# vincentjzy/OpenCorr

Hardware: AMD Instinct MI355X
Metric: converged POIs/sec (FFTCC+ICGN2D1, 33x33 subset) (higher is better)
Workload: dtype f32

## Files before the change

opencorr_amd/csrc/capi.hip:

```cpp
#include "capi_internal.h"

namespace ochip_capi {

thread_local std::string g_last_error;

int fail(int code, const char* fmt, ...) {
    char buf[512];
    va_list ap;
    va_start(ap, fmt);
    vsnprintf(buf, sizeof(buf), fmt, ap);
    va_end(ap);
    g_last_error = buf;
    return code;
}

static std::once_flag g_rocfft_once;
void rocfft_init_once() {
    std::call_once(g_rocfft_once, [] { rocfft_setup(); });
}

int create_engine(int kind, int rx, int ry, int rz, float conv, float stop, int device, oc_hip_engine** out) {
    if (!out) return fail(OC_HIP_ERR_INVALID, "null output handle");
    *out = nullptr;
    if (rx < 1 || ry < 1 || ((kind == OC_HIP_FFTCC3D || kind == OC_HIP_ICGN3D1) && rz < 1))
        return fail(OC_HIP_ERR_INVALID, "subset radius must be >= 1 (got %d, %d, %d)", rx, ry, rz);
    int ndev = 0;
    hipError_t err = hipGetDeviceCount(&ndev);
    if (err != hipSuccess || ndev <= 0)
        return fail(OC_HIP_ERR_HIP, "no usable HIP device: %s", err == hipSuccess ? "device count is 0" : hipGetErrorString(err));
    if (device < 0 || device >= ndev) return fail(OC_HIP_ERR_INVALID, "device %d out of range [0,%d)", device, ndev);
    DeviceScope device_scope;
    OC_HIP_TRY(hipSetDevice(device));
    std::unique_ptr<oc_hip_engine> e(new oc_hip_engine);
    e->kind = kind;
    e->device = device;
    e->rx = rx;
    e->ry = ry;
    e->rz = rz;
    e->conv = conv;
    e->stop = stop;
    OC_HIP_TRY(hipStreamCreateWithFlags(&e->own_stream, hipStreamNonBlocking));
    e->stream = e->own_stream;
    *out = e.release();
    return OC_HIP_OK;
}

}

namespace {

size_t fftcc_chunk_limit() {
#if OC_BUILD_AB
    const char* s = getenv("OC_HIP_FFTCC_CHUNK");
    if (s && *s) {
        long v = atol(s);
        if (v > 0) return (size_t)v;
    }
#endif
    return 32768;
}

int ensure_fft(oc_hip_engine* e, size_t chunk) {
    const int n0 = 2 * e->rx, n1 = 2 * e->ry, n2 = e->is3d() ? 2 * e->rz : 0;
    FftPlans& f = e->fft;
    if (f.fwd && f.n0 == n0 && f.n1 == n1 && f.n2 == n2 && f.chunk == chunk) return OC_HIP_OK;
    rocfft_init_once();
    f.destroy();
    const size_t lengths2[2] = {(size_t)n1, (size_t)n0};
    const size_t lengths3[3] = {(size_t)n2, (size_t)n1, (size_t)n0};
    const size_t* lengths = n2 ? lengths3 : lengths2;
    const size_t dims = n2 ? 3 : 2;
    OC_FFT_TRY(rocfft_plan_create(&f.fwd, rocfft_placement_notinplace, rocfft_transform_type_real_forward,
                                  rocfft_precision_single, dims, lengths, 2 * chunk, nullptr));
    OC_FFT_TRY(rocfft_plan_create(&f.inv, rocfft_placement_notinplace, rocfft_transform_type_real_inverse,
                                  rocfft_precision_single, dims, lengths, chunk, nullptr));
    OC_FFT_TRY(rocfft_execution_info_create(&f.info_fwd));
    OC_FFT_TRY(rocfft_execution_info_create(&f.info_inv));
    size_t wf = 0, wi = 0;
    OC_FFT_TRY(rocfft_plan_get_work_buffer_size(f.fwd, &wf));
    OC_FFT_TRY(rocfft_plan_get_work_buffer_size(f.inv, &wi));
    if (wf) {
        OC_TRY(f.work_fwd.reserve(wf));
        OC_FFT_TRY(rocfft_execution_info_set_work_buffer(f.info_fwd, f.work_fwd.p, wf));
    }
    if (wi) {
        OC_TRY(f.work_inv.reserve(wi));
        OC_FFT_TRY(rocfft_execution_info_set_work_buffer(f.info_inv, f.work_inv.p, wi));
    }
    f.n0 = n0;
    f.n1 = n1;
    f.n2 = n2;
    f.chunk = chunk;
    return OC_HIP_OK;
}

int run_fftcc2d(oc_hip_engine* e, float* d_pois, int stride_f, size_t count) {
    if (!e->img || e->img->ndim != 2) return fail(OC_HIP_ERR_INVALID, "FFTCC2D: set_images2d has not been called");
    const ImagePair& im = *e->img;
    const bool fused32 = e->fftcc2d_fused != 2 && ochip::fftcc2d_fused_supported(e->rx, e->ry);
    const bool rect = ochip::fftcc2d_rect_supported(e->rx, e->ry);
    if (e->fftcc2d_fused && (fused32 || rect || ochip::fftcc2d_fusedn_supported(e->rx, e->ry))) {
        ochip::Fftcc2dParams P = {im.ref_ptr(), im.tar_ptr(), im.dy, im.dx, e->rx, e->ry};
        ProfScope prof(e);
        const size_t kMaxBatch = 1u << 30;
        for (size_t first = 0; first < count; first += kMaxBatch) {
            const size_t n = (count - first) < kMaxBatch ? (count - first) : kMaxBatch;
            float* q = d_pois + first * (size_t)stride_f;
            hipError_t err = fused32 ? ochip::launch_fftcc2d_fused(P, q, stride_f, n, e->icgn2d_xcd != 0, e->stream)
                             : rect  ? ochip::launch_fftcc2d_rect(P, q, stride_f, n, e->icgn2d_xcd != 0, e->stream)
                                     : ochip::launch_fftcc2d_fusedn(P, q, stride_f, n, e->icgn2d_xcd != 0, e->stream);
            if (err != hipSuccess) return fail(OC_HIP_ERR_HIP, "fused FFTCC2D launch failed: %s", hipGetErrorString(err));
        }
        return OC_HIP_OK;
    }
    const size_t chunk = count < fftcc_chunk_limit() ? count : fftcc_chunk_limit();
    if (chunk == 0) return OC_HIP_OK;
    OC_TRY(ensure_fft(e, chunk));
    const size_t M = (size_t)4 * e->rx * e->ry;
    const size_t F = (size_t)(2 * e->rx) * (size_t)(e->ry + 1);
    OC_TRY(e->win.reserve(2 * chunk * M * sizeof(float)));
    OC_TRY(e->freq.reserve(2 * chunk * F * sizeof(float2)));
    OC_TRY(e->norms.reserve(2 * chunk * sizeof(float)));
    OC_TRY(e->flags.reserve(chunk * sizeof(int)));
    OC_FFT_TRY(rocfft_execution_info_set_stream(e->fft.info_fwd, e->stream));
    OC_FFT_TRY(rocfft_execution_info_set_stream(e->fft.info_inv, e->stream));
    ochip::Fftcc2dParams P = {im.ref_ptr(), im.tar_ptr(), im.dy, im.dx, e->rx, e->ry};
    float* ref_win = e->win.as<float>();
    float* tar_win = ref_win + chunk * M;
    float2* ref_freq = e->freq.as<float2>();
    float2* tar_freq = ref_freq + chunk * F;
    ProfScope prof(e);
    for (size_t first = 0; first < count; first += chunk) {
        const size_t n = (count - first) < chunk ? (count - first) : chunk;
        float* pois = d_pois + first * (size_t)stride_f;
        if (n < chunk) {
            OC_HIP_TRY(hipMemsetAsync(ref_win + n * M, 0, (chunk - n) * M * sizeof(float), e->stream));
            OC_HIP_TRY(hipMemsetAsync(tar_win + n * M, 0, (chunk - n) * M * sizeof(float), e->stream));
        }
        OC_HIP_TRY(ochip::launch_fftcc2d_gather(P, pois, stride_f, n, ref_win, tar_win, e->norms.as<float>(),
                                                e->flags.as<int>(), e->stream));
        void* in_fwd[1] = {ref_win};
        void* out_fwd[1] = {ref_freq};
        OC_FFT_TRY(rocfft_execute(e->fft.fwd, in_fwd, out_fwd, e->fft.info_fwd));
        OC_HIP_TRY(ochip::launch_fftcc_conjmul(ref_freq, tar_freq, ref_freq, n * F, e->stream));
        void* in_inv[1] = {ref_freq};
        void* out_inv[1] = {ref_win};
        OC_FFT_TRY(rocfft_execute(e->fft.inv, in_inv, out_inv, e->fft.info_inv));
        OC_HIP_TRY(ochip::launch_fftcc2d_argmax(P, ref_win, e->norms.as<float>(), e->flags.as<int>(), pois, stride_f,
                                                n, e->stream));
    }
    return OC_HIP_OK;
}

int tile_order(oc_hip_engine* e, const float* pois, int stride_f, size_t n, const unsigned** perm, unsigned* xy_copy = nullptr,
               unsigned* xy_word = nullptr, unsigned xy_epoch = 0) {
    *perm = nullptr;
    if (e->icgn2d_tile_px <= 0 || n < 16384) {
        if (xy_copy) OC_HIP_TRY(ochip::launch_poi2d_xy_check(pois, stride_f, n, xy_copy, xy_word, xy_epoch, e->stream));
        return OC_HIP_OK;
    }
    const ImagePair& im = *e->img;
    OC_TRY(e->perm.reserve(n * sizeof(unsigned)));
    OC_TRY(e->tiles.reserve(ochip::poi2d_tile_count(im.dy, im.dx, e->icgn2d_tile_px) * sizeof(unsigned)));
    OC_TRY(e->perm_slots.reserve(n * sizeof(unsigned)));
    OC_HIP_TRY(ochip::launch_poi2d_tile_order(pois, stride_f, n, im.dy, im.dx, e->icgn2d_tile_px, e->tiles.as<unsigned>(),
                                              e->perm_slots.as<unsigned>(), e->perm.as<unsigned>(), e->stream, xy_copy, xy_word, xy_epoch));
    *perm = e->perm.as<unsigned>();
    return OC_HIP_OK;
}

int check_image2d_limits(const char* who, const ImagePair& im, unsigned long long max_pixels) {
    if ((unsigned long long)im.dy * (unsigned long long)im.dx > max_pixels || im.dx >= (1 << 22) || im.dy >= (1 << 22))
        return fail(OC_HIP_ERR_UNSUPPORTED, "%s: image %d x %d exceeds the engine's limit of %llu pixels (width, height < 2^22)", who,
                    im.dx, im.dy, max_pixels);
    return OC_HIP_OK;
}

int run_icgn2d(oc_hip_engine* e, float* d_pois, int stride_f, size_t count, const float* d_offsets) {
    if (!e->img || e->img->ndim != 2) return fail(OC_HIP_ERR_INVALID, "ICGN2D: set_images2d has not been called");
    if (!e->ref_ready || !e->tar_ready)
        return fail(OC_HIP_ERR_INVALID, "ICGN2D: prepare() has not been called since the last set_images");
    const ImagePair& im = *e->img;
    OC_TRY(check_image2d_limits("ICGN2D", im, 1ull << 28));
    const int dof = (e->kind == OC_HIP_ICGN2D1 || e->kind == OC_HIP_ICLM2D1) ? 6 : 12;
    const bool lm = e->is_iclm();
    const bool onepass = e->arith_onepass && !lm;
    if (onepass && d_offsets)
        return fail(OC_HIP_ERR_UNSUPPORTED, "ICGN2D%d: centre offsets are not supported under arith_onepass = 1 (the one-pass kernel keeps "
                                            "integer local coordinates in a per-workgroup table); set arith_onepass = 0 for this call", dof == 6 ? 1 : 2);
    if (onepass && e->self_adaptive)
        return fail(OC_HIP_ERR_UNSUPPORTED, "ICGN2D%d: self-adaptive subset radii are not supported under arith_onepass = 1 (the one-pass "
// ... 736 lines not shown
        }
        if (e->switch_ev && hipEventRecord(e->switch_ev, e->own_stream) == hipSuccess) have_event = true;
        else (void)hipStreamSynchronize(e->own_stream);
    } else {
        have_event = e->tail_marked && e->switch_ev;
    }
    if (have_event && next != e->own_stream) {
        const hipError_t err = hipStreamWaitEvent(next, e->switch_ev, 0);
        if (err != hipSuccess) {
            (void)hipGetLastError();
            return fail(OC_HIP_ERR_HIP, "set_stream: cannot enqueue on the new stream: %s", hipGetErrorString(err));
        }
    } else if (have_event) {
        if (hipStreamWaitEvent(e->own_stream, e->switch_ev, 0) != hipSuccess) {
            (void)hipGetLastError();
            (void)hipEventSynchronize(e->switch_ev);
            (void)hipGetLastError();
        }
    }
    (void)must_succeed;
    e->stream = next;
    e->tail_marked = have_event;
    return OC_HIP_OK;
}

int oc_hip_set_stream(oc_hip_engine* e, void* hip_stream) {
    OC_ACTIVATE(e);
    std::lock_guard<std::mutex> lock(e->mu);
    return switch_stream(e, reinterpret_cast<hipStream_t>(hip_stream), false);
}

int oc_hip_reset_stream(oc_hip_engine* e) {
    OC_ACTIVATE(e);
    std::lock_guard<std::mutex> lock(e->mu);
    return switch_stream(e, e->own_stream, true);
}

int oc_hip_set_tuning(oc_hip_engine* e, const char* key, int value) {
    OC_TRY(check_engine(e));
    if (!key) return fail(OC_HIP_ERR_INVALID, "null tuning key");
    std::lock_guard<std::mutex> lock(e->mu);
    const std::string k(key);
    if (k == "icgn2d_variant") {
        if (value < -1 || value >= ochip::icgn2d_variant_count())
            return fail(OC_HIP_ERR_INVALID, "icgn2d_variant %d out of range [-1 (automatic), %d)", value, ochip::icgn2d_variant_count());
        if (value >= 0 && !ochip::icgn2d_variant_built(value))
            return fail(OC_HIP_ERR_UNSUPPORTED, "icgn2d_variant %d is an A/B partner that only the A/B build of the library contains "
                                               "(python -m opencorr_amd.build --ab)", value);
        e->icgn2d_variant = value;
    } else if (k == "icgn2d_xcd" || k == "xcd") {
        e->icgn2d_xcd = value != 0;
    } else if (k == "arith_fma") {
        if (value != 0 && !(e->is_icgn2d() || e->kind == OC_HIP_ICGN3D1))
            return fail(OC_HIP_ERR_UNSUPPORTED, "arith_fma: only the ICGN2D1 / ICGN2D2 / ICLM2D1 / ICLM2D2 / ICGN3D1 engines have a fused-arithmetic build");
        e->arith_fma = value != 0;
    } else if (k == "arith_onepass") {
        if (value != 0 && e->kind == OC_HIP_ICGN3D1)
            return fail(OC_HIP_ERR_UNSUPPORTED, "arith_onepass: the key of the ICGN2D1 / ICGN2D2 engines; the one-pass build of ICGN3D1 has a "
                                                "key of its own, arith_onepass3d");
        if (value != 0 && !(e->kind == OC_HIP_ICGN2D1 || e->kind == OC_HIP_ICGN2D2))
            return fail(OC_HIP_ERR_UNSUPPORTED, "arith_onepass: only the ICGN2D1 / ICGN2D2 engines have a one-pass build");
        e->arith_onepass = value != 0;
    } else if (k == "arith_onepass3d") {
        if (value != 0 && e->kind != OC_HIP_ICGN3D1)
            return fail(OC_HIP_ERR_UNSUPPORTED, "arith_onepass3d: only the ICGN3D1 engine has this one-pass build (ICGN2D1 / ICGN2D2: "
                                                "arith_onepass)");
        e->arith_onepass3d = value != 0;
    } else if (k == "icgn2d_split_chunks") {
#if !OC_BUILD_AB
        if (value != 0)
            return fail(OC_HIP_ERR_UNSUPPORTED, "icgn2d_split_chunks belongs to icgn2d_variant 8, an A/B partner that only the A/B build of the "
                                                "library contains (python -m opencorr_amd.build --ab)");
#endif
        if (value < 0 || value > 256) return fail(OC_HIP_ERR_INVALID, "icgn2d_split_chunks must be 0 (back to back) ... 256");
        e->icgn2d_split_chunks = value;
    } else if (k == "icgn2d_setup_cache") {
        e->icgn2d_setup_cache = value != 0;
    } else if (k == "icgn2d_int_first") {
        e->icgn2d_int_first = value != 0;
    } else if (k == "icgn2d_tile_px") {
        if (value < 0 || (value > 0 && value < 16)) return fail(OC_HIP_ERR_INVALID, "icgn2d_tile_px must be 0 (off) or >= 16");
        e->icgn2d_tile_px = value;
    } else if (k == "fftcc2d_fused") {
        e->fftcc2d_fused = value == 2 ? 2 : (value != 0);
    } else if (k == "fftcc3d_fused") {
#if !OC_BUILD_AB
        if (value == 2)
            return fail(OC_HIP_ERR_UNSUPPORTED, "fftcc3d_fused = 2 (the 32^3 kernel of rounds 1 - 5) is an A/B partner that only the A/B build of the "
                                                "library contains (python -m opencorr_amd.build --ab)");
#endif
        e->fftcc3d_fused = value == 2 ? 2 : (value != 0);
    } else if (k == "fftcc3d_tile_vox") {
        if (value < 0 || (value > 0 && value < 8)) return fail(OC_HIP_ERR_INVALID, "fftcc3d_tile_vox must be 0 (off) or >= 8");
        e->fftcc3d_tile_vox = value;
    } else if (k == "icgn3d_tile_vox") {
        if (value < 0 || (value > 0 && value < 8)) return fail(OC_HIP_ERR_INVALID, "icgn3d_tile_vox must be 0 (off) or >= 8");
        e->icgn3d_tile_vox = value;
    } else if (k == "icgn3d_mapping") {
#if !OC_BUILD_AB
        if (value != 0)
            return fail(OC_HIP_ERR_UNSUPPORTED, "icgn3d_mapping = 1 (the row mapping, measured 12 - 25 %% slower) is an A/B partner that only "
                                               "the A/B build of the library contains (python -m opencorr_amd.build --ab)");
#endif
        e->icgn3d_mapping = value != 0;
    } else if (k == "fftcc3d_planes_blocks") {
        if (value < 0 || value > 4096) return fail(OC_HIP_ERR_INVALID, "fftcc3d_planes_blocks must be 0 (default) ... 4096");
        e->fftcc3d_planes_blocks = value;
    } else if (k == "single_combine") {
        e->single_combine = value != 0;
    } else if (k == "host_chunk") {
        if (value < 0 || (value > 0 && value < 16384)) return fail(OC_HIP_ERR_INVALID, "host_chunk must be 0 (off) or >= 16384 POIs");
        e->host_chunk = value;
    } else if (k == "group_allgather") {
        e->group_allgather = value != 0;
    } else if (k == "group_force_rccl") {
        e->group_force_rccl = value != 0;
    } else {
        return fail(OC_HIP_ERR_INVALID, "unknown tuning key '%s'", key);
    }
    for (oc_hip_engine* r : e->replicas) OC_TRY(oc_hip_set_tuning(r, key, value));
    return OC_HIP_OK;
}

int oc_hip_prepare_ref(oc_hip_engine* e) {
    OC_ACTIVATE(e);
    if (!e->is_icgn()) return OC_HIP_OK;
    if (!e->img) return fail(OC_HIP_ERR_INVALID, "prepare: set_images has not been called");
    std::lock_guard<std::mutex> lock(e->mu);
    TailGuard tail(e);
    OC_TRY(order_after_default_stream(e));
    const ImagePair& im = *e->img;
    const size_t bytes = im.count() * sizeof(float);
    if (e->kind == OC_HIP_NR2D1) {
        e->ref_ready = true;
        for (oc_hip_engine* r : e->replicas) OC_TRY(oc_hip_prepare_ref(r));
        return OC_HIP_OK;
    }
    if (im.ndim == 2) {
        OC_TRY(e->gx.reserve(bytes));
        OC_TRY(e->gy.reserve(bytes));
        OC_HIP_TRY(ochip::launch_grad2d(im.ref_ptr(), im.dy, im.dx, e->gx.as<float>(), e->gy.as<float>(), e->stream));
    } else {
        OC_TRY(e->gx.reserve(bytes));
        OC_TRY(e->gy.reserve(bytes));
        OC_TRY(e->gz.reserve(bytes));
        OC_HIP_TRY(ochip::launch_grad3d(im.ref_ptr(), im.dz, im.dy, im.dx, e->gx.as<float>(), e->gy.as<float>(),
                                        e->gz.as<float>(), e->stream));
    }
    e->ref_ready = true;
    e->ref_generation++;
    OC_TRY(mark_tail(e));
    for (oc_hip_engine* r : e->replicas) OC_TRY(oc_hip_prepare_ref(r));
    OC_HIP_TRY(hipSetDevice(e->device));
    return OC_HIP_OK;
}

int oc_hip_prepare_tar(oc_hip_engine* e) {
    OC_ACTIVATE(e);
    if (!e->is_icgn()) return OC_HIP_OK;
    if (!e->img) return fail(OC_HIP_ERR_INVALID, "prepare: set_images has not been called");
    std::lock_guard<std::mutex> lock(e->mu);
    TailGuard tail(e);
    OC_TRY(order_after_default_stream(e));
    const ImagePair& im = *e->img;
    if (im.ndim == 2) {
        OC_TRY(check_image2d_limits(e->kind == OC_HIP_NR2D1 ? "NR2D1" : "ICGN2D", im, e->kind == OC_HIP_NR2D1 ? 1ull << 26 : 1ull << 28));
        const bool with_val = e->kind == OC_HIP_ICGN2D1 || e->kind == OC_HIP_ICGN2D2;
// ... 413 lines not shown
```

opencorr_amd/csrc/fft_device.h:

```cpp
#pragma once

#include <hip/hip_runtime.h>

#include <type_traits>

#define OC_FFT_FN __host__ __device__ __forceinline__

namespace ochip {
namespace fftdev {

__device__ constexpr float kCos16[8] = {1.000000000e+00f, 9.238795325e-01f, 7.071067812e-01f, 3.826834324e-01f, 6.123233996e-17f, -3.826834324e-01f, -7.071067812e-01f, -9.238795325e-01f};
__device__ constexpr float kSin16[8] = {0.000000000e+00f, 3.826834324e-01f, 7.071067812e-01f, 9.238795325e-01f, 1.000000000e+00f, 9.238795325e-01f, 7.071067812e-01f, 3.826834324e-01f};
__device__ constexpr float kCos32[16] = {1.000000000e+00f, 9.807852804e-01f, 9.238795325e-01f, 8.314696123e-01f, 7.071067812e-01f, 5.555702330e-01f, 3.826834324e-01f, 1.950903220e-01f, 6.123233996e-17f, -1.950903220e-01f, -3.826834324e-01f, -5.555702330e-01f, -7.071067812e-01f, -8.314696123e-01f, -9.238795325e-01f, -9.807852804e-01f};
__device__ constexpr float kSin32[16] = {0.000000000e+00f, 1.950903220e-01f, 3.826834324e-01f, 5.555702330e-01f, 7.071067812e-01f, 8.314696123e-01f, 9.238795325e-01f, 9.807852804e-01f, 1.000000000e+00f, 9.807852804e-01f, 9.238795325e-01f, 8.314696123e-01f, 7.071067812e-01f, 5.555702330e-01f, 3.826834324e-01f, 1.950903220e-01f};

typedef float c2 __attribute__((ext_vector_type(2)));
OC_FFT_FN c2 mkc(float re, float im) {
    c2 r = {re, im};
    return r;
}

template <bool INV>
OC_FFT_FN c2 cmul_tw(c2 d, float c, float s) {
#pragma clang fp contract(fast)
// ... 242 lines not shown
    const c2 p14 = a1 + a4, m14 = a1 - a4, p23 = a2 + a3, m23 = a2 - a3;
    const c2 r1 = a0 + p14 * c1 + p23 * c2_, r2 = a0 + p14 * c2_ + p23 * c1;
    const c2 i1 = rot90<INV>(m14 * s1 + m23 * s2), i2 = rot90<INV>(m14 * s2 - m23 * s1);
    a0 = a0 + p14 + p23;
    a1 = r1 + i1;
    a4 = r1 - i1;
    a2 = r2 + i2;
    a3 = r2 - i2;
}

template <bool INV, int P, int OFF, int M, int LEN>
OC_FFT_FN void dft_prime(c2 (&v)[LEN]) {
#pragma clang fp contract(fast)
    constexpr int H = (P - 1) / 2;
    c2 ps[H], ms[H];
    static_for<0, H>([&](auto jc) {
        constexpr int j = decltype(jc)::value;
        const c2 a = v[OFF + (j + 1) * M], b = v[OFF + (P - 1 - j) * M];
        ps[j] = a + b;
        ms[j] = a - b;
    });
    const c2 a0 = v[OFF];
    c2 total = a0;
    static_for<0, H>([&](auto jc) { total = total + ps[decltype(jc)::value]; });
    static_for<1, H + 1>([&](auto kc) {
        constexpr int k = decltype(kc)::value;
        c2 re = a0, im = mkc(0.f, 0.f);
        static_for<0, H>([&](auto jc) {
            constexpr int j = decltype(jc)::value;
            constexpr int idx = ((j + 1) * k) % P;
            constexpr float cc = Twiddle<P>::c[idx], ss = Twiddle<P>::s[idx];
            re = re + ps[j] * cc;
            im = im + ms[j] * ss;
        });
        const c2 ri = rot90<INV>(im);
        v[OFF + k * M] = re + ri;
        v[OFF + (P - k) * M] = re - ri;
    });
    v[OFF] = total;
}

template <bool INV, int TOP, int M, int OFF, int LEN, int S, int R>
OC_FFT_FN void fft_mixed_blocks(c2 (&v)[LEN]);

template <bool INV, int TOP, int N, int OFF, int LEN>
OC_FFT_FN void fft_mixed_at(c2 (&v)[LEN]) {
    if constexpr (N > 1) {
        constexpr int R = fft_radix(N), M = N / R;
        static_assert(R <= kFftMaxPrime, "window side must factor into primes <= 31");
        static_for<0, M>([&](auto n2c) {
            constexpr int n2 = decltype(n2c)::value;
            if constexpr (R == 2) dft2<INV>(v[OFF + n2], v[OFF + n2 + M]);
            if constexpr (R == 3) dft3<INV>(v[OFF + n2], v[OFF + n2 + M], v[OFF + n2 + 2 * M]);
            if constexpr (R == 4) dft4<INV>(v[OFF + n2], v[OFF + n2 + M], v[OFF + n2 + 2 * M], v[OFF + n2 + 3 * M]);
            if constexpr (R == 5)
                dft5<INV>(v[OFF + n2], v[OFF + n2 + M], v[OFF + n2 + 2 * M], v[OFF + n2 + 3 * M], v[OFF + n2 + 4 * M]);
            if constexpr (R > 5) dft_prime<INV, R, OFF + n2, M, LEN>(v);
            if constexpr (n2 != 0) {
                static_for<1, R>([&](auto sc) {
                    constexpr int s = decltype(sc)::value;
                    constexpr int m = (n2 * s) % N * (TOP / N);
                    constexpr float tc = Twiddle<TOP>::c[m], ts = Twiddle<TOP>::s[m];
                    v[OFF + n2 + s * M] = cmul_tw<INV>(v[OFF + n2 + s * M], tc, ts);
                });
            }
        });
        fft_mixed_blocks<INV, TOP, M, OFF, LEN, 0, R>(v);
    }
}

template <bool INV, int TOP, int M, int OFF, int LEN, int S, int R>
OC_FFT_FN void fft_mixed_blocks(c2 (&v)[LEN]) {
    if constexpr (S < R) {
        fft_mixed_at<INV, TOP, M, OFF + S * M, LEN>(v);
        fft_mixed_blocks<INV, TOP, M, OFF, LEN, S + 1, R>(v);
    }
}

template <bool INV, int N>
OC_FFT_FN void fft_mixed(c2 (&v)[N]) {
    fft_mixed_at<INV, N, N, 0, N>(v);
}

}
}
```

opencorr_amd/csrc/fftcc2d_fused.hip:

```cpp
#include "dic2d_device.h"
#include "fft_device.h"
#include "oc_kernels.h"

namespace ochip {

namespace {

using namespace fftdev;

constexpr int FN = 32;
constexpr int FP = FN + 1;
constexpr int FWAVE_LDS = FN * FP;
#ifndef OC_FFTCC2D_X2
#define OC_FFTCC2D_X2 1
#endif
#if !OC_FFTCC2D_X2
#ifndef OC_FFTCC2D_WAVES
#define OC_FFTCC2D_WAVES 4
#endif
constexpr int kFusedWaves = OC_FFTCC2D_WAVES;

template <bool INV>
__device__ __forceinline__ void fft32_line(const c2* line, int step, int h, c2 (&v)[16]) {
#pragma clang fp contract(fast)
// ... 66 lines not shown
        }
        rn = wave_allreduce_sum(rn);
        tn = wave_allreduce_sum(tn);
    }
    __builtin_amdgcn_wave_barrier();

    const int line = lane & 31, h = lane >> 5;
    c2 v[16];
    fft32_line<false>(buf + line * FP, 1, h, v);
    __builtin_amdgcn_wave_barrier();
#pragma unroll
    for (int k = 0; k < 16; k++) buf[line * FP + 2 * k + h] = v[bitrev4(k)];
    __builtin_amdgcn_wave_barrier();
    fft32_line<false>(buf + line, FP, h, v);
    __builtin_amdgcn_wave_barrier();
#pragma unroll
    for (int k = 0; k < 16; k++) buf[(2 * k + h) * FP + line] = v[bitrev4(k)];
    __builtin_amdgcn_wave_barrier();
    {
        const int mx = (FN - line) & (FN - 1);
        c2 zm[16];
#pragma unroll
        for (int k = 0; k < 16; k++) zm[k] = buf[((FN - (2 * k + h)) & (FN - 1)) * FP + mx];
        __builtin_amdgcn_wave_barrier();
#pragma unroll
        for (int k = 0; k < 16; k++) {
            const c2 z = v[bitrev4(k)];
            const float rr = 0.5f * (z.x + zm[k].x), ri = 0.5f * (z.y - zm[k].y);
            const float tr = 0.5f * (z.y + zm[k].y), ti = -0.5f * (z.x - zm[k].x);
            buf[(2 * k + h) * FP + line] = mkc((rr * tr) + (ri * ti), (rr * ti) - (ri * tr));
        }
    }
    __builtin_amdgcn_wave_barrier();
    fft32_line<true>(buf + line * FP, 1, h, v);
    __builtin_amdgcn_wave_barrier();
#pragma unroll
    for (int k = 0; k < 16; k++) buf[line * FP + 2 * k + h] = v[bitrev4(k)];
    __builtin_amdgcn_wave_barrier();
    fft32_line<true>(buf + line, FP, h, v);

    float best = -2.f;
    int bidx = 0;
#pragma unroll
    for (int k = 0; k < 16; k++) {
        const float val = v[bitrev4(k)].x;
        if (val > best) { best = val; bidx = (2 * k + h) * FN + line; }
    }
#pragma unroll
    for (int off = 1; off < kWave; off <<= 1) {
        const float ov = __shfl_xor(best, off, kWave);
        const int oi = __shfl_xor(bidx, off, kWave);
        if (ov > best || (ov == best && oi < bidx)) { best = ov; bidx = oi; }
    }
    if (lane == 0) {
        int du = bidx % FN, dv = bidx / FN;
        if (du > rx) du -= FN;
        if (dv > ry) dv -= FN;
        poi[poi2d::U] = (float)du + gu;
        poi[poi2d::V] = (float)dv + gv;
        poi[poi2d::U0] = gu;
        poi[poi2d::V0] = gv;
        poi[poi2d::ZNCC] = best / (sqrtf(rn * tn) * M);
    }
}
#endif

#ifndef OC_FFTCC2D_X2_WAVES
#define OC_FFTCC2D_X2_WAVES 1
#endif
#ifndef OC_FFTCC2D_X2_SPLIT
#define OC_FFTCC2D_X2_SPLIT 1
#endif
#ifndef OC_FFTCC2D_X2_OCC
#define OC_FFTCC2D_X2_OCC (OC_FFTCC2D_X2_SPLIT ? 4 : 2)
#endif
constexpr int kX2Waves = OC_FFTCC2D_X2_WAVES;

__device__ __forceinline__ float half_wave_sum(float v) {
#pragma unroll
    for (int off = 1; off < 32; off <<= 1) v += __shfl_xor(v, off, kWave);
    return v;
}

__global__ __launch_bounds__(64 * kX2Waves, OC_FFTCC2D_X2_OCC) void fftcc2d_fused32x2_kernel(Fftcc2dParams P, float* __restrict__ pois, int stride_f,
                                                                         unsigned long long count, int xcd_chunk) {
    __shared__ c2 lds[kX2Waves * 2 * FWAVE_LDS / (OC_FFTCC2D_X2_SPLIT ? 2 : 1)];
    const int lane = threadIdx.x & (kWave - 1);
    const int wave = __builtin_amdgcn_readfirstlane(threadIdx.x >> 6);
    const int q = lane >> 5, l = lane & 31;
    unsigned long long grp = blockIdx.x;
    if (xcd_chunk > 0) grp = (unsigned long long)(blockIdx.x & 7u) * xcd_chunk + (blockIdx.x >> 3);
    const unsigned long long idx = (grp * kX2Waves + wave) * 2 + q;
    if (idx >= count) return;
    c2* tile = lds + (wave * 2 + q) * (FWAVE_LDS / (OC_FFTCC2D_X2_SPLIT ? 2 : 1));
    float* poi = pois + idx * (unsigned long long)stride_f;
    const float px = poi[poi2d::X], py = poi[poi2d::Y];
    const float gu = poi[poi2d::U], gv = poi[poi2d::V];
    const int rx = FN / 2, ry = FN / 2, width = P.width, height = P.height;
    constexpr int M = FN * FN;
    if ((int)px < rx || (int)px >= width - rx || (int)py < ry || (int)py >= height - ry || (int)(px + gu) < rx ||
        (int)(px + gu) >= width - rx || (int)(py + gv) < ry || (int)(py + gv) >= height - ry)
        return;

    c2 v[FN];
    float rn, tn;
    {
        const __amdgpu_buffer_rsrc_t r_ref = make_rsrc(P.ref), r_tar = make_rsrc(P.tar);
        const float rxp = px + l - rx, txp = rxp + gu;
#pragma unroll
        for (int k = 0; k < FN; k++) {
            const float ryp = py + k - ry, typ = ryp + gv;
            const float a = buf_f32(r_ref, (__umul24((unsigned)(int)ryp, (unsigned)width) + (unsigned)(int)rxp) << 2, 0);
            const float b = buf_f32(r_tar, (__umul24((unsigned)(int)typ, (unsigned)width) + (unsigned)(int)txp) << 2, 0);
            v[k] = mkc(a, b);
        }
        float rsum = 0.f, tsum = 0.f;
#pragma unroll
        for (int k = 0; k < FN; k++) {
            rsum += v[k].x;
            tsum += v[k].y;
        }
        const c2 mean = mkc(half_wave_sum(rsum) / M, half_wave_sum(tsum) / M);
        rn = 0.f;
        tn = 0.f;
#pragma unroll
        for (int k = 0; k < FN; k++) {
            v[k] = v[k] - mean;
            rn += v[k].x * v[k].x;
            tn += v[k].y * v[k].y;
        }
        rn = half_wave_sum(rn);
        tn = half_wave_sum(tn);
        asm volatile("" : "+v"(rn), "+v"(tn));
    }
    fft32<false>(v);
#if OC_FFTCC2D_X2_SPLIT
    float* __restrict__ ft = reinterpret_cast<float*>(tile);
#define OC_X2_TRANSPOSE(WRITE_IDX, READ_IDX)                                                   \
    _Pragma("unroll") for (int k = 0; k < FN; k++) ft[WRITE_IDX] = v[bitrev5(k)].x;            \
    __builtin_amdgcn_wave_barrier();                                                           \
    _Pragma("unroll") for (int k = 0; k < FN; k++) v[k].x = ft[READ_IDX];                      \
    __builtin_amdgcn_wave_barrier();                                                           \
    _Pragma("unroll") for (int k = 0; k < FN; k++) ft[WRITE_IDX] = v[bitrev5(k)].y;            \
    __builtin_amdgcn_wave_barrier();                                                           \
    _Pragma("unroll") for (int k = 0; k < FN; k++) v[k].y = ft[READ_IDX];                      \
    __builtin_amdgcn_wave_barrier();
#else
#define OC_X2_TRANSPOSE(WRITE_IDX, READ_IDX)                                                   \
    _Pragma("unroll") for (int k = 0; k < FN; k++) tile[WRITE_IDX] = v[bitrev5(k)];            \
    __builtin_amdgcn_wave_barrier();                                                           \
    _Pragma("unroll") for (int k = 0; k < FN; k++) v[k] = tile[READ_IDX];                      \
    __builtin_amdgcn_wave_barrier();
#endif
    OC_X2_TRANSPOSE(k * FP + l, l * FP + k)
    fft32<false>(v);
    {
        const int mrow = ((FN - l) & (FN - 1)) * FP;
        auto product = [](c2 z, c2 zm) {
            const float rr = z.x + zm.x, ri = z.y - zm.y;
            const float tr = z.y + zm.y, ti = zm.x - z.x;
            return mkc((rr * tr) + (ri * ti), (rr * ti) - (ri * tr));
        };
#if OC_FFTCC2D_X2_SPLIT
        float zmx[FN];
#pragma unroll
        for (int k = 0; k < FN; k++) ft[l * FP + k] = v[bitrev5(k)].x;
        __builtin_amdgcn_wave_barrier();
#pragma unroll
        for (int k = 0; k < FN; k++) zmx[k] = ft[mrow + ((FN - k) & (FN - 1))];
        __builtin_amdgcn_wave_barrier();
#pragma unroll
        for (int k = 0; k < FN; k++) ft[l * FP + k] = v[bitrev5(k)].y;
        __builtin_amdgcn_wave_barrier();
#pragma unroll
        for (int k = 0; k < FN; k++) v[bitrev5(k)] = product(v[bitrev5(k)], mkc(zmx[k], ft[mrow + ((FN - k) & (FN - 1))]));
        __builtin_amdgcn_wave_barrier();
#else
#pragma unroll
        for (int k = 0; k < FN; k++) tile[l * FP + k] = v[bitrev5(k)];
        __builtin_amdgcn_wave_barrier();
#pragma unroll
        for (int k = 0; k < FN; k++) v[bitrev5(k)] = product(v[bitrev5(k)], tile[mrow + ((FN - k) & (FN - 1))]);
        __builtin_amdgcn_wave_barrier();
#endif
    }
    c2 u[FN];
#pragma unroll
    for (int k = 0; k < FN; k++) u[k] = v[bitrev5(k)];
    fft32<true>(u);
#pragma unroll
    for (int k = 0; k < FN; k++) v[k] = u[k];
    OC_X2_TRANSPOSE(l * FP + k, k * FP + l)
#undef OC_X2_TRANSPOSE
#pragma unroll
    for (int k = 0; k < FN; k++) u[k] = v[k];
    fft32<true>(u);

    float best = -2.f;
    int bidx = 0;
#pragma unroll
    for (int r = 0; r < FN; r++) {
        const float val = u[bitrev5(r)].x;
        if (val > best) { best = val; bidx = r * FN + l; }
    }
#pragma unroll
    for (int off = 1; off < 32; off <<= 1) {
        const float ov = __shfl_xor(best, off, kWave);
        const int oi = __shfl_xor(bidx, off, kWave);
        if (ov > best || (ov == best && oi < bidx)) { best = ov; bidx = oi; }
    }
    if (l == 0) {
        if (rn == 0.f || tn == 0.f) {
            best = 0.f;
            bidx = 0;
        }
        int du = bidx % FN, dv = bidx / FN;
        if (du > rx) du -= FN;
        if (dv > ry) dv -= FN;
        poi[poi2d::U] = (float)du + gu;
        poi[poi2d::V] = (float)dv + gv;
        poi[poi2d::U0] = gu;
        poi[poi2d::V0] = gv;
        poi[poi2d::ZNCC] = (0.25f * best) / (sqrtf(rn * tn) * M);
    }
}

bool fftcc2d_fused_supported(int rx, int ry) { return rx == FN / 2 && ry == FN / 2; }

hipError_t launch_fftcc2d_fused(const Fftcc2dParams& p, float* pois, int stride_f, size_t count, bool xcd,
                                hipStream_t stream) {
    if (count == 0) return hipSuccess;
    if (!fftcc2d_fused_supported(p.rx, p.ry)) return hipErrorInvalidValue;
    (void)hipGetLastError();
#if OC_FFTCC2D_X2
    {
        const size_t groups = (count + 2 * kX2Waves - 1) / (2 * kX2Waves);
        const int chunk = xcd ? (int)((groups + 7) / 8) : 0;
        const size_t grid = xcd ? (size_t)chunk * 8 : groups;
        hipLaunchKernelGGL(fftcc2d_fused32x2_kernel, dim3((unsigned)grid), dim3(64 * kX2Waves), 0, stream, p, pois, stride_f,
                           (unsigned long long)count, chunk);
        return hipGetLastError();
    }
#else
    const size_t groups = (count + kFusedWaves - 1) / kFusedWaves;
    const int chunk = xcd ? (int)((groups + 7) / 8) : 0;
    const size_t grid = xcd ? (size_t)chunk * 8 : groups;
    hipLaunchKernelGGL(fftcc2d_fused32_kernel, dim3((unsigned)grid), dim3(64 * kFusedWaves), 0, stream, p, pois, stride_f,
                       (unsigned long long)count, chunk);
    return hipGetLastError();
#endif
}

}
```

opencorr_amd/csrc/oc_kernels.h:

```cpp
#pragma once

#include <hip/hip_runtime.h>
#include <stddef.h>

#ifndef OC_BUILD_AB
#define OC_BUILD_AB 0
#endif

namespace ochip {

hipError_t launch_grad2d(const float* img, int height, int width, float* gx, float* gy, hipStream_t stream);
hipError_t launch_bspline2d_lut(const float* img, int height, int width, float* lut, hipStream_t stream, float* value_plane = nullptr);
hipError_t launch_colmajor_to_rowmajor(const float* src, int height, int width, float* dst, hipStream_t stream);

struct Icgn2dParams {
    const float* ref;
    const float* gx;
    const float* gy;
    const float* lut;
    int height, width;
    int rx, ry;
    float conv, stop;
    const float* offsets;
    const unsigned* perm;
// ... 108 lines not shown
    const float* map_x;
    const float* map_y;
    int height, width;
    float proj[12];
};
hipError_t launch_undistort_map(const CameraParams& cam, int height, int width, float convergence, int iteration, float* map_x,
                                float* map_y, hipStream_t stream);
hipError_t launch_undistort_points(const CameraView& view, const float* in, float* out, int stride_floats, size_t count,
                                   hipStream_t stream);
hipError_t launch_reconstruct(const CameraView& view1, const CameraView& view2, const float* p1, int stride1_floats,
                              const float* p2, int stride2_floats, float* out, int stride_out_floats, size_t count,
                              hipStream_t stream);
hipError_t launch_reconstruct_pois(const CameraView& view1, const CameraView& view2, float* pois, int stride_floats, size_t count,
                                   hipStream_t stream);

hipError_t launch_poi2d_best_of_segments(const float* cand, int cand_stride_floats, const unsigned* seg_start, size_t nseg,
                                         float* pois, int stride_floats, hipStream_t stream);

struct Nr2dParams {
    const float* ref;
    const float* lut;
    const float* lut_gx;
    const float* lut_gy;
    int height, width;
    int rx, ry;
    float conv, stop;
    const unsigned* perm;
};
hipError_t launch_nr2d1(const Nr2dParams& p, float* pois, int stride_floats, size_t count, hipStream_t stream);
int nr2d1_max_samples();

hipError_t launch_grad3d(const float* vol, int dz, int dy, int dx, float* gx, float* gy, float* gz, hipStream_t stream);
hipError_t launch_bspline3d_prefilter(const float* vol, int dz, int dy, int dx, float* coef, float* tmp,
                                      hipStream_t stream);

struct Icgn3dParams {
    const float* ref;
    const float* gx;
    const float* gy;
    const float* gz;
    const float* coef;
    int dz, dy, dx;
    int rx, ry, rz;
    float conv, stop;
    float* scratch;
    int samples_per_pass;
    int tail_steps_per_pass;
    const unsigned* perm;
    int arith_fma;
};
size_t icgn3d1_scratch_floats(int rx, int ry, int rz, int* blocks);
hipError_t launch_icgn3d1(const Icgn3dParams& p, float* pois, int stride_floats, size_t count, hipStream_t stream);
namespace sep {
hipError_t launch_icgn3d1(const Icgn3dParams& p, float* pois, int stride_floats, size_t count, hipStream_t stream);
}
namespace fma {
hipError_t launch_icgn3d1(const Icgn3dParams& p, float* pois, int stride_floats, size_t count, hipStream_t stream);
}
hipError_t launch_icgn3d1_onepass(const Icgn3dParams& p, float* pois, int stride_floats, size_t count, hipStream_t stream);
size_t icgn3d1_rows_slot_floats(int rx, int ry, int rz);
hipError_t launch_icgn3d1_rows(const Icgn3dParams& p, float* pois, int stride_floats, size_t count, int blocks, hipStream_t stream);

struct Fftcc2dParams {
    const float* ref;
    const float* tar;
    int height, width;
    int rx, ry;
};
hipError_t launch_fftcc2d_gather(const Fftcc2dParams& p, const float* pois, int stride_floats, size_t count,
                                 float* ref_win, float* tar_win, float* norms, int* flags, hipStream_t stream);
hipError_t launch_fftcc_conjmul(const float2* rf, const float2* tf, float2* zf, size_t bins, hipStream_t stream);
hipError_t launch_fftcc2d_argmax(const Fftcc2dParams& p, const float* surf, const float* norms, const int* flags,
                                 float* pois, int stride_floats, size_t count, hipStream_t stream);

bool fftcc2d_fusedn_supported(int rx, int ry);
hipError_t launch_fftcc2d_fusedn(const Fftcc2dParams& p, float* pois, int stride_floats, size_t count, bool xcd,
                                 hipStream_t stream);

bool fftcc2d_rect_supported(int rx, int ry);
hipError_t launch_fftcc2d_rect(const Fftcc2dParams& p, float* pois, int stride_floats, size_t count, bool xcd, hipStream_t stream);

bool fftcc2d_fused_supported(int rx, int ry);
hipError_t launch_fftcc2d_fused(const Fftcc2dParams& p, float* pois, int stride_floats, size_t count, bool xcd,
                                hipStream_t stream);

struct Fftcc3dParams {
    const float* ref;
    const float* tar;
    int dz, dy, dx;
    int rx, ry, rz;
    const unsigned* perm = nullptr;
};
hipError_t launch_fftcc3d_gather(const Fftcc3dParams& p, const float* pois, int stride_floats, size_t count,
                                 float* ref_win, float* tar_win, float* norms, hipStream_t stream);
hipError_t launch_fftcc3d_argmax(const Fftcc3dParams& p, const float* surf, const float* norms, float* pois,
                                 int stride_floats, size_t count, hipStream_t stream);

bool fftcc3d_fused_supported(int rx, int ry, int rz);
hipError_t launch_fftcc3d_fused(const Fftcc3dParams& p, float* pois, int stride_floats, size_t count, bool xcd, hipStream_t stream);
#if OC_BUILD_AB
size_t fftcc3d_fused_flag_bytes(size_t count);
hipError_t launch_fftcc3d_fused_r5(const Fftcc3dParams& p, float* pois, int stride_floats, size_t count, bool xcd,
                                   unsigned char* needs_clamped, hipStream_t stream);
#endif

bool fftcc3d_fusedn_supported(int rx, int ry, int rz);
hipError_t launch_fftcc3d_fusedn(const Fftcc3dParams& p, float* pois, int stride_floats, size_t count, bool xcd,
                                 hipStream_t stream);

bool fftcc3d_box_supported(int rx, int ry, int rz);
hipError_t launch_fftcc3d_box(const Fftcc3dParams& p, float* pois, int stride_floats, size_t count, bool xcd, hipStream_t stream);

bool fftcc3d_planes_supported(int rx, int ry, int rz);
size_t fftcc3d_planes_scratch_bytes(int radius, int blocks);
hipError_t launch_fftcc3d_planes(const Fftcc3dParams& p, float* pois, int stride_floats, size_t count, void* scratch, int blocks,
                                 hipStream_t stream);

struct PoiSplitParams {
    int mode;
    int rec_floats;
    int zncc_at, conv_at;
    float zncc_low, zncc_high, conv;
};
hipError_t launch_poi_index_range(const unsigned* index, size_t n, size_t limit, unsigned* flag, hipStream_t stream);
size_t poi_split_scratch_words(size_t count);
hipError_t launch_poi_split(const float* pois, int stride_floats, size_t count, const PoiSplitParams& p, const unsigned* index_in,
                            float* out0, size_t out0_offset, unsigned* index_out0, float* out1, unsigned* index_out,
                            float* main_queue, size_t main_count, unsigned* scratch, hipStream_t stream);

}
```

Before: 82.07 million.

## Use Hermitian half-size inverse FFT and strided row loads in fused FFTCC2D

After: 83.34 million, median of 6. 1.02x the previous value.

```diff
diff --git a/opencorr_amd/csrc/capi.hip b/opencorr_amd/csrc/capi.hip
--- a/opencorr_amd/csrc/capi.hip
+++ b/opencorr_amd/csrc/capi.hip
@@ -106,7 +106,7 @@
         for (size_t first = 0; first < count; first += kMaxBatch) {
             const size_t n = (count - first) < kMaxBatch ? (count - first) : kMaxBatch;
             float* q = d_pois + first * (size_t)stride_f;
-            hipError_t err = fused32 ? ochip::launch_fftcc2d_fused(P, q, stride_f, n, e->icgn2d_xcd != 0, e->stream)
+            hipError_t err = fused32 ? ochip::launch_fftcc2d_fused(P, q, stride_f, n, e->icgn2d_xcd != 0, e->stream, e->fftcc2d_fused)
                              : rect  ? ochip::launch_fftcc2d_rect(P, q, stride_f, n, e->icgn2d_xcd != 0, e->stream)
                                      : ochip::launch_fftcc2d_fusedn(P, q, stride_f, n, e->icgn2d_xcd != 0, e->stream);
             if (err != hipSuccess) return fail(OC_HIP_ERR_HIP, "fused FFTCC2D launch failed: %s", hipGetErrorString(err));
@@ -1009,7 +1009,7 @@
         if (value < 0 || (value > 0 && value < 16)) return fail(OC_HIP_ERR_INVALID, "icgn2d_tile_px must be 0 (off) or >= 16");
         e->icgn2d_tile_px = value;
     } else if (k == "fftcc2d_fused") {
-        e->fftcc2d_fused = value == 2 ? 2 : (value != 0);
+        e->fftcc2d_fused = (value >= 2 && value <= 5) ? value : (value != 0);
     } else if (k == "fftcc3d_fused") {
 #if !OC_BUILD_AB
         if (value == 2)
diff --git a/opencorr_amd/csrc/fft_device.h b/opencorr_amd/csrc/fft_device.h
--- a/opencorr_amd/csrc/fft_device.h
+++ b/opencorr_amd/csrc/fft_device.h
@@ -348,5 +348,22 @@
     fft_mixed_at<INV, N, N, 0, N>(v);
 }
 
-}
-}
+template <int LEN>
+OC_FFT_FN void ifft32_hermitian(const c2 (&X)[LEN], c2 (&z)[16]) {
+    static_assert(LEN >= 17, "needs X[0 .. 16]");
+    z[0] = mkc(X[0].x + X[16].x, X[0].x - X[16].x);
+    z[8] = mkc(X[8].x + X[8].x, -(X[8].y + X[8].y));
+    static_for<1, 8>([&](auto kc) {
+        constexpr int k = decltype(kc)::value;
+        constexpr float tc = Twiddle<32>::c[k], ts = Twiddle<32>::s[k];
+        const c2 p = X[k], q = mkc(X[16 - k].x, -X[16 - k].y);
+        const c2 s = p + q;
+        const c2 t = cmul_tw<true>(p - q, tc, ts);
+        z[k] = mkc(s.x - t.y, s.y + t.x);
+        z[16 - k] = mkc(s.x + t.y, t.x - s.y);
+    });
+    fft_mixed_at<true, 16, 16, 0, 16>(z);
+}
+
+}
+}
diff --git a/opencorr_amd/csrc/fftcc2d_fused.hip b/opencorr_amd/csrc/fftcc2d_fused.hip
--- a/opencorr_amd/csrc/fftcc2d_fused.hip
+++ b/opencorr_amd/csrc/fftcc2d_fused.hip
@@ -172,6 +172,7 @@
     return v;
 }
 
+template <bool FAST_ROWS, bool REAL_LAST>
 __global__ __launch_bounds__(64 * kX2Waves, OC_FFTCC2D_X2_OCC) void fftcc2d_fused32x2_kernel(Fftcc2dParams P, float* __restrict__ pois, int stride_f,
                                                                          unsigned long long count, int xcd_chunk) {
     __shared__ c2 lds[kX2Waves * 2 * FWAVE_LDS / (OC_FFTCC2D_X2_SPLIT ? 2 : 1)];
@@ -197,12 +198,22 @@
     {
         const __amdgpu_buffer_rsrc_t r_ref = make_rsrc(P.ref), r_tar = make_rsrc(P.tar);
         const float rxp = px + l - rx, txp = rxp + gu;
-#pragma unroll
-        for (int k = 0; k < FN; k++) {
-            const float ryp = py + k - ry, typ = ryp + gv;
-            const float a = buf_f32(r_ref, (__umul24((unsigned)(int)ryp, (unsigned)width) + (unsigned)(int)rxp) << 2, 0);
-            const float b = buf_f32(r_tar, (__umul24((unsigned)(int)typ, (unsigned)width) + (unsigned)(int)txp) << 2, 0);
-            v[k] = mkc(a, b);
+        const bool integral = px == (float)(int)px && py == (float)(int)py && gu == (float)(int)gu && gv == (float)(int)gv;
+        if (FAST_ROWS && __builtin_amdgcn_ballot_w64(!integral) == 0) {
+            const float ry0 = py - ry, ty0 = ry0 + gv;
+            const unsigned ref0 = (__umul24((unsigned)(int)ry0, (unsigned)width) + (unsigned)(int)rxp) << 2;
+            const unsigned tar0 = (__umul24((unsigned)(int)ty0, (unsigned)width) + (unsigned)(int)txp) << 2;
+            const unsigned pitch = (unsigned)width << 2;
+#pragma unroll
+            for (int k = 0; k < FN; k++) v[k] = mkc(buf_f32(r_ref, ref0, k * pitch), buf_f32(r_tar, tar0, k * pitch));
+        } else {
+#pragma unroll
+            for (int k = 0; k < FN; k++) {
+                const float ryp = py + k - ry, typ = ryp + gv;
+                const float a = buf_f32(r_ref, (__umul24((unsigned)(int)ryp, (unsigned)width) + (unsigned)(int)rxp) << 2, 0);
+                const float b = buf_f32(r_tar, (__umul24((unsigned)(int)typ, (unsigned)width) + (unsigned)(int)txp) << 2, 0);
+                v[k] = mkc(a, b);
+            }
         }
         float rsum = 0.f, tsum = 0.f;
 #pragma unroll
@@ -280,19 +291,48 @@
     fft32<true>(u);
 #pragma unroll
     for (int k = 0; k < FN; k++) v[k] = u[k];
-    OC_X2_TRANSPOSE(l * FP + k, k * FP + l)
-#undef OC_X2_TRANSPOSE
-#pragma unroll
-    for (int k = 0; k < FN; k++) u[k] = v[k];
-    fft32<true>(u);
-
     float best = -2.f;
     int bidx = 0;
-#pragma unroll
-    for (int r = 0; r < FN; r++) {
-        const float val = u[bitrev5(r)].x;
-        if (val > best) { best = val; bidx = r * FN + l; }
-    }
+    if constexpr (REAL_LAST) {
+#if OC_FFTCC2D_X2_SPLIT
+#pragma unroll
+        for (int k = 0; k < FN; k++) ft[l * FP + k] = v[bitrev5(k)].x;
+        __builtin_amdgcn_wave_barrier();
+#pragma unroll
+        for (int k = 0; k <= FN / 2; k++) v[k].x = ft[k * FP + l];
+        __builtin_amdgcn_wave_barrier();
+#pragma unroll
+        for (int k = 0; k < FN; k++) ft[l * FP + k] = v[bitrev5(k)].y;
+        __builtin_amdgcn_wave_barrier();
+#pragma unroll
+        for (int k = 0; k <= FN / 2; k++) v[k].y = ft[k * FP + l];
+#else
+#pragma unroll
+        for (int k = 0; k < FN; k++) tile[l * FP + k] = v[bitrev5(k)];
+        __builtin_amdgcn_wave_barrier();
+#pragma unroll
+        for (int k = 0; k <= FN / 2; k++) v[k] = tile[k * FP + l];
+#endif
+        c2 z[FN / 2];
+        ifft32_hermitian(v, z);
+        static_for<0, FN>([&](auto rc) {
+            constexpr int r = decltype(rc)::value;
+            constexpr int pos = fft_pos(FN / 2, r >> 1);
+            const float val = (r & 1) ? z[pos].y : z[pos].x;
+            if (val > best) { best = val; bidx = r * FN + l; }
+        });
+    } else {
+        OC_X2_TRANSPOSE(l * FP + k, k * FP + l)
+#pragma unroll
+        for (int k = 0; k < FN; k++) u[k] = v[k];
+        fft32<true>(u);
+#pragma unroll
+        for (int r = 0; r < FN; r++) {
+            const float val = u[bitrev5(r)].x;
+            if (val > best) { best = val; bidx = r * FN + l; }
+        }
+    }
+#undef OC_X2_TRANSPOSE
 #pragma unroll
     for (int off = 1; off < 32; off <<= 1) {
         const float ov = __shfl_xor(best, off, kWave);
@@ -318,7 +358,7 @@
 bool fftcc2d_fused_supported(int rx, int ry) { return rx == FN / 2 && ry == FN / 2; }
 
 hipError_t launch_fftcc2d_fused(const Fftcc2dParams& p, float* pois, int stride_f, size_t count, bool xcd,
-                                hipStream_t stream) {
+                                hipStream_t stream, int body) {
     if (count == 0) return hipSuccess;
     if (!fftcc2d_fused_supported(p.rx, p.ry)) return hipErrorInvalidValue;
     (void)hipGetLastError();
@@ -327,7 +367,11 @@
         const size_t groups = (count + 2 * kX2Waves - 1) / (2 * kX2Waves);
         const int chunk = xcd ? (int)((groups + 7) / 8) : 0;
         const size_t grid = xcd ? (size_t)chunk * 8 : groups;
-        hipLaunchKernelGGL(fftcc2d_fused32x2_kernel, dim3((unsigned)grid), dim3(64 * kX2Waves), 0, stream, p, pois, stride_f,
+        auto kern = body == 3 ? fftcc2d_fused32x2_kernel<false, false>
+                    : body == 4 ? fftcc2d_fused32x2_kernel<true, false>
+                    : body == 5 ? fftcc2d_fused32x2_kernel<false, true>
+                                : fftcc2d_fused32x2_kernel<true, true>;
+        hipLaunchKernelGGL(kern, dim3((unsigned)grid), dim3(64 * kX2Waves), 0, stream, p, pois, stride_f,
                            (unsigned long long)count, chunk);
         return hipGetLastError();
     }
diff --git a/opencorr_amd/csrc/oc_kernels.h b/opencorr_amd/csrc/oc_kernels.h
--- a/opencorr_amd/csrc/oc_kernels.h
+++ b/opencorr_amd/csrc/oc_kernels.h
@@ -214,7 +214,7 @@
 
 bool fftcc2d_fused_supported(int rx, int ry);
 hipError_t launch_fftcc2d_fused(const Fftcc2dParams& p, float* pois, int stride_floats, size_t count, bool xcd,
-                                hipStream_t stream);
+                                hipStream_t stream, int body = 1);
 
 struct Fftcc3dParams {
     const float* ref;
```
